# kjedrzejewski/video-cycle_gan-upscaling

Hardware: AMD Instinct MI355X
Metric: upscaled frames/s (train step, G+D fwd+bwd) at 256->512 (higher is better)
Workload: dtype f32; 1 GPU; C2: make_upscaler_orig((512,512,3),k=3,x2,res=9) + PatchGAN-70, batch 8/GPU, gan2 wiring, Wasserstein + pixel-MSE, faithful 3-call step incl. predict pass; global_batch=8, frame=256x256->512x512, parallelism=dp1, launch=hipGraph replay

## Files before the change

### video-cycle_gan-upscaling_amd/csrc/conv_wgrad.hip

```cpp
#include "vcg_common.hpp"

namespace {

struct WgradParams {
    const float* A;
    const float* B;
    float* part;
    float* dbpart;
    int n, mtot, ah, aw;
    int jctot, bh, bw;
    int pt, pl, flip;
    int jc;
    int m_blocks, j_blocks, slabs;
    int tiles_x, tiles_y, tiles_total, tiles_per_slab;
    int m_pad, j_pad;
};

template <int S, int NW, int NJ, int MW, int TH, int KH, int KW>
struct WgCfg {
    static constexpr int T = KH * KW;
    static constexpr int NT = 64 * NW;
    static constexpr int JTILES = (MW == 2 ? NW : NW / 2) * NJ;
    static constexpr int JCMAX = (JTILES * 32) / T;
    static constexpr int AST = TH * 32 + 1;
    static constexpr int BH = (TH - 1) * S + KH;
    static constexpr int BW = 31 * S + KW;
    static constexpr int round_to(int v, int r) { return v + ((r - v % 32) % 32 + 32) % 32; }
    static constexpr int BRS = round_to(BW, KW % 32);
    static constexpr int BPS = round_to(BH * BRS, T % 32);
    static constexpr int A_ELEMS = 64 * TH * 32;
    static constexpr int B_ELEMS = JCMAX * BH * BW;
    static constexpr int A_PT = (A_ELEMS + NT - 1) / NT;
    static constexpr int RG = NT / 32;
    static constexpr int ROWS = JCMAX * BH;
    static constexpr int QSEG = BW / 32, REM = BW % 32;
    static constexpr int RPT = (ROWS + RG - 1) / RG;
    static constexpr int HPT = (ROWS * REM + NT - 1) / NT;
    static constexpr int REMD = REM > 0 ? REM : 1;
    static constexpr int B_PT = RPT * QSEG + HPT;
    static constexpr size_t LDS_BYTES = ((size_t)64 * AST + (size_t)JCMAX * BPS + 64) * sizeof(float);
};

template <int S, int NW, int NJ, int MW, int TH, int KH, int KW>
__global__ __launch_bounds__(64 * NW, (MW * NJ * 16 > 100 ? 1 : 2)) void wgrad_kernel(const WgradParams p) {
    using C = WgCfg<S, NW, NJ, MW, TH, KH, KW>;
    extern __shared__ __attribute__((aligned(16))) float smem[];
    float* s_a = smem;
    float* s_b = smem + 64 * C::AST;

    const int tid = threadIdx.x, lane = tid & 63, wv = tid >> 6;
    const int half = lane >> 5, l31 = lane & 31;
    int b = blockIdx.x;
    const int jb = b % p.j_blocks; b /= p.j_blocks;
    const int mb = b % p.m_blocks; b /= p.m_blocks;
    const int slab = b;
    const int m0 = mb * 64, jc0 = jb * p.jc;
    const int jc_here = min(p.jc, p.jctot - jc0);
    const int jvalid = jc_here * C::T;

    int boff[NJ];
#pragma unroll
    for (int i = 0; i < NJ; ++i) {
        const int j = ((MW == 2 ? wv : (wv >> 1)) * NJ + i) * 32 + l31;
        int o = 0;
        if (j < jvalid) {
            const int jc = j / C::T, t = j % C::T;
            int ky = t / KW, kx = t % KW;
            if (p.flip) { ky = KH - 1 - ky; kx = KW - 1 - kx; }
            o = jc * C::BPS + ky * C::BRS + kx;
        }
        boff[i] = o + half * S;
    }
    const float* ap0 = s_a + ((MW == 2 ? 0 : (wv & 1)) * 32 + l31) * C::AST + half;

    f32x16 acc[MW][NJ];
#pragma unroll
    for (int m = 0; m < MW; ++m)
#pragma unroll
        for (int i = 0; i < NJ; ++i)
#pragma unroll
            for (int r = 0; r < 16; ++r) acc[m][i][r] = 0.f;
    float dbacc = 0.f;
    const bool do_db = p.dbpart != nullptr && jb == 0 && wv == 0;

    const int t_begin = slab * p.tiles_per_slab;
    const int t_end = min(t_begin + p.tiles_per_slab, p.tiles_total);

    float ra[C::A_PT], rb[C::B_PT];
    auto load_tile = [&](int tile) {
        int q = tile;
        const int tx = q % p.tiles_x; q /= p.tiles_x;
        const int ty = q % p.tiles_y; q /= p.tiles_y;
        const int n = q;
        const int ax0 = tx * 32, ay0 = ty * TH;
        const vcg_rsrc rA = make_rsrc(p.A + (size_t)n * p.mtot * p.ah * p.aw, (size_t)p.mtot * p.ah * p.aw * sizeof(float));
#pragma unroll
        for (int i = 0; i < C::A_PT; ++i) {
            const int e = tid + i * C::NT;
            const int c = e & 31, r = (e >> 5) % TH, m = e / (32 * TH);
            const int ay = ay0 + r, ax = ax0 + c;
            const bool ok = e < C::A_ELEMS && m0 + m < p.mtot && ay < p.ah && ax < p.aw;
            ra[i] = buf_load(rA, ok ? 4u * (unsigned)(((m0 + m) * p.ah + ay) * p.aw + ax) : VCG_OOB);
        }
        const vcg_rsrc rB = make_rsrc(p.B + ((size_t)n * p.jctot + jc0) * p.bh * p.bw, (size_t)(p.jctot - jc0) * p.bh * p.bw * sizeof(float));
        const int by0 = ay0 * S - p.pt, bx0 = ax0 * S - p.pl;
        const int c32 = tid & 31, rg = tid >> 5;
#pragma unroll
        for (int i = 0; i < C::RPT; ++i) {
            const int row = rg + i * C::RG;
            const int jc = row / C::BH, r = row % C::BH;
            const int by = by0 + r;
            const bool rok = row < C::ROWS && jc < jc_here && by >= 0 && by < p.bh;
            const int rbase = (jc * p.bh + by) * p.bw + bx0;
#pragma unroll
            for (int q = 0; q < C::QSEG; ++q) {
                const int bx = bx0 + q * 32 + c32;
                const bool ok = rok && bx >= 0 && bx < p.bw;
                rb[i * C::QSEG + q] = buf_load(rB, ok ? 4u * (unsigned)(rbase + q * 32 + c32) : VCG_OOB);
            }
        }
#pragma unroll
        for (int i = 0; i < C::HPT; ++i) {
            const int e = tid + i * C::NT;
            const int row = e / C::REMD, c = C::QSEG * 32 + e % C::REMD;
            const int jc = row / C::BH, r = row % C::BH;
            const int by = by0 + r, bx = bx0 + c;
            const bool ok = row < C::ROWS && jc < jc_here && by >= 0 && by < p.bh && bx >= 0 && bx < p.bw;
            rb[C::RPT * C::QSEG + i] = buf_load(rB, ok ? 4u * (unsigned)((jc * p.bh + by) * p.bw + bx) : VCG_OOB);
        }
    };
    auto store_tile = [&]() {
#pragma unroll
        for (int i = 0; i < C::A_PT; ++i) {
            const int e = tid + i * C::NT;
            if (e < C::A_ELEMS) {
                const int c = e & 31, r = (e >> 5) % TH, m = e / (32 * TH);
                s_a[m * C::AST + r * 32 + c] = ra[i];
            }
        }
        const int c32 = tid & 31, rg = tid >> 5;
#pragma unroll
        for (int i = 0; i < C::RPT; ++i) {
            const int row = rg + i * C::RG;
            if (row < C::ROWS) {
                const int jc = row / C::BH, r = row % C::BH;
#pragma unroll
                for (int q = 0; q < C::QSEG; ++q) s_b[jc * C::BPS + r * C::BRS + q * 32 + c32] = rb[i * C::QSEG + q];
            }
        }
#pragma unroll
        for (int i = 0; i < C::HPT; ++i) {
            const int e = tid + i * C::NT;
            const int row = e / C::REMD, c = C::QSEG * 32 + e % C::REMD;
            if (row < C::ROWS) {
                const int jc = row / C::BH, r = row % C::BH;
                s_b[jc * C::BPS + r * C::BRS + c] = rb[C::RPT * C::QSEG + i];
            }
        }
    };

    if (t_begin < t_end) load_tile(t_begin);
    for (int tile = t_begin; tile < t_end; ++tile) {
        __syncthreads();
        store_tile();
        __syncthreads();
        if (tile + 1 < t_end) load_tile(tile + 1);
        if (do_db) {
            const float* row = s_a + lane * C::AST;
#pragma unroll
            for (int i = 0; i < TH * 32; ++i) dbacc += row[i];
        }
#pragma unroll
        for (int r = 0; r < TH; ++r) {
#pragma unroll
            for (int st = 0; st < 16; ++st) {
                float av[MW];
#pragma unroll
                for (int m = 0; m < MW; ++m) av[m] = ap0[m * 32 * C::AST + r * 32 + 2 * st];
#pragma unroll
                for (int i = 0; i < NJ; ++i) {
                    const float bv = s_b[boff[i] + (r * S) * C::BRS + 2 * st * S];
#pragma unroll
                    for (int m = 0; m < MW; ++m) acc[m][i] = mfma32(av[m], bv, acc[m][i]);
                }
            }
        }
    }

    float* out = p.part + ((size_t)slab * p.m_pad + m0 + (MW == 2 ? 0 : (wv & 1)) * 32) * p.j_pad + (size_t)jb * (C::JTILES * 32);
#pragma unroll
    for (int m = 0; m < MW; ++m)
#pragma unroll
        for (int i = 0; i < NJ; ++i) {
            const int jcol = ((MW == 2 ? wv : (wv >> 1)) * NJ + i) * 32 + l31;
#pragma unroll
            for (int r = 0; r < 16; ++r) out[(size_t)(m * 32 + mfma_row(r, lane)) * p.j_pad + jcol] = acc[m][i][r];
        }
    if (do_db) p.dbpart[(size_t)slab * p.m_pad + m0 + lane] = dbacc;
}

struct ReduceParams {
    const float* part;
    const float* dbpart;
    float* dw;
    float* db;
    int slabs, m_pad, j_pad, mtot, jctot, jc, jbw, T;
    int ts, sm, sj;
};

__global__ __launch_bounds__(256) void wgrad_reduce_kernel(const ReduceParams p) {
    const size_t idx = (size_t)blockIdx.x * 256 + threadIdx.x;
    const size_t total = (size_t)p.m_pad * p.j_pad;
    if (idx >= total) return;
    const int m = (int)(idx / p.j_pad), jg = (int)(idx % p.j_pad);
    if (m >= p.mtot) return;
    const int jb = jg / p.jbw, jl = jg % p.jbw;
    if (jl >= p.jc * p.T) return;
    const int jc = jb * p.jc + jl / p.T, t = jl % p.T;
    if (jc >= p.jctot) return;
    float s8[8] = {0.f, 0.f, 0.f, 0.f, 0.f, 0.f, 0.f, 0.f};
    const float* src = p.part + idx;
    int k = 0;
    for (; k + 8 <= p.slabs; k += 8) {
#pragma unroll
        for (int u = 0; u < 8; ++u) s8[u] += src[(size_t)(k + u) * total];
    }
#pragma unroll
    for (int u = 0; u < 8; ++u)
        if (k + u < p.slabs) s8[u] += src[(size_t)(k + u) * total];
    const float s = ((s8[0] + s8[1]) + (s8[2] + s8[3])) + ((s8[4] + s8[5]) + (s8[6] + s8[7]));
    p.dw[(size_t)t * p.ts + (size_t)m * p.sm + (size_t)jc * p.sj] = s;
}

__global__ __launch_bounds__(256) void wgrad_db_reduce_kernel(const float* dbpart, float* db, int slabs, int m_pad, int mtot) {
    __shared__ float red[4][64];
    const int c = threadIdx.x & 63, g = threadIdx.x >> 6;
    const int m = blockIdx.x * 64 + c;
    float s4[4] = {0.f, 0.f, 0.f, 0.f};
    if (m < mtot) {
        int k = g;
        for (; k + 12 < slabs; k += 16) {
#pragma unroll
            for (int u = 0; u < 4; ++u) s4[u] += dbpart[(size_t)(k + 4 * u) * m_pad + m];
        }
        for (; k < slabs; k += 4) s4[0] += dbpart[(size_t)k * m_pad + m];
    }
    red[g][c] = (s4[0] + s4[1]) + (s4[2] + s4[3]);
    __syncthreads();
    if (g == 0 && m < mtot) db[m] = (red[0][c] + red[1][c]) + (red[2][c] + red[3][c]);
}

struct Plan {
    int S, NW, NJ, MW, TH, KH, KW, jc, m_blocks, j_blocks, slabs, tiles_x, tiles_y, tiles_total, tiles_per_slab;
    int m_pad, j_pad;
    size_t ws_part_bytes, ws_bytes;
    bool ok;
};

inline void pick_layout(int KH, int KW, int S, int jtot, int* nw, int* nj, int* mw) {
    *mw = 2;
    if (jtot <= 64) { *nw = 2; *nj = 1; return; }
    if (KH != KW) { *nw = 4; *nj = 2; return; }
    switch (KH) {
        case 1: *nw = 4; *nj = 2; return;
        case 3: if (jtot <= 256) { *nw = 4; *nj = 2; } else { *nw = 4; *nj = 9; *mw = 1; } return;
        case 4: if (S == 2) { *nw = 4; *nj = 2; } else { *nw = 4; *nj = 8; *mw = 1; } return;
        case 5: if (jtot <= 256 || S == 3) { *nw = 4; *nj = 2; } else { *nw = 4; *nj = 13; *mw = 1; } return;
        case 9: *nw = 4; *nj = 2; return;
        default: *nw = 0; *nj = 0; return;
    }
}

Plan make_plan(int n, int mtot, int ah, int aw, int jctot, int kh, int kw, int S) {
    Plan pl{};
    pl.ok = false;
    if (S < 1 || S > 3 || (S == 3 && (kh != 5 || kw != 5)) || (kh == 9 && S != 1)) return pl;
    if (kh != kw && (S != 1 || (kh != 1 && kw != 1))) return pl;
    if (kh == 1 && kw == 1 && S != 1) return pl;
    const int T = kh * kw;
    pl.S = S; pl.KH = kh; pl.KW = kw;
    pl.TH = (S == 1) ? 2 : 1;
    pick_layout(kh, kw, S, jctot * T, &pl.NW, &pl.NJ, &pl.MW);
    if (pl.NW == 0) return pl;
    const int cap = (pl.MW == 2 ? pl.NW : pl.NW / 2) * pl.NJ * 32;
    pl.jc = cap / T;
    if (pl.jc < 1) return pl;
    if (pl.jc > jctot) pl.jc = jctot;
    pl.m_blocks = ceil_div(mtot, 64);
    pl.j_blocks = ceil_div(jctot, pl.jc);
    pl.tiles_x = ceil_div(aw, 32);
    pl.tiles_y = ceil_div(ah, pl.TH);
    pl.tiles_total = pl.tiles_x * pl.tiles_y * n;
    int slabs = ceil_div(pl.MW == 1 ? 256 : 768, pl.m_blocks * pl.j_blocks);
    if (slabs > pl.tiles_total) slabs = pl.tiles_total;
    if (slabs < 1) slabs = 1;
    pl.tiles_per_slab = ceil_div(pl.tiles_total, slabs);
    pl.slabs = ceil_div(pl.tiles_total, pl.tiles_per_slab);
    pl.m_pad = pl.m_blocks * 64;
    pl.j_pad = pl.j_blocks * cap;
    pl.ws_part_bytes = align_up((size_t)pl.slabs * pl.m_pad * pl.j_pad * sizeof(float), 256);
    pl.ws_bytes = pl.ws_part_bytes + (size_t)pl.slabs * pl.m_pad * sizeof(float);
    pl.ok = true;
    return pl;
}

template <int S, int NW, int NJ, int MW, int TH, int KH, int KW>
int launch_wgrad(const WgradParams& p, int grid, hipStream_t st) {
    using C = WgCfg<S, NW, NJ, MW, TH, KH, KW>;
    static_assert(C::LDS_BYTES <= 160 * 1024, "wgrad tile does not fit the 160 KiB LDS");
    auto kern = wgrad_kernel<S, NW, NJ, MW, TH, KH, KW>;
    if (int e = vcg_allow_dyn_lds(reinterpret_cast<const void*>(kern), C::LDS_BYTES)) return e;
    hipLaunchKernelGGL(kern, dim3(grid), dim3(C::NT), C::LDS_BYTES, st, p);
    VCG_LAUNCH_CHECK();
    return VCG_OK;
}

}

size_t vcg_internal_wgrad_ws(int n, int mtot, int ah, int aw, int jctot, int kh, int kw, int S) {
    Plan pl = make_plan(n, mtot, ah, aw, jctot, kh, kw, S);
    return pl.ok ? pl.ws_bytes : 0;
}

int vcg_internal_wgrad(const float* A, const float* B, float* dw, float* db, int n, int mtot, int ah, int aw,
                       int jctot, int bh, int bw, int kh, int kw, int S, int pt, int pl_, int flip, int ts, int sm,
                       int sj, void* ws, size_t ws_bytes, hipStream_t st) {
    Plan pl = make_plan(n, mtot, ah, aw, jctot, kh, kw, S);
    if (!pl.ok) return VCG_E_UNSUPPORTED;
    if (ws == nullptr || ws_bytes < pl.ws_bytes) return VCG_E_WORKSPACE;
    WgradParams p{};
    p.A = A; p.B = B; p.part = (float*)ws;
    p.dbpart = db ? (float*)((char*)ws + pl.ws_part_bytes) : nullptr;
    p.n = n; p.mtot = mtot; p.ah = ah; p.aw = aw; p.jctot = jctot; p.bh = bh; p.bw = bw;
    p.pt = pt; p.pl = pl_; p.flip = flip; p.jc = pl.jc;
    p.m_blocks = pl.m_blocks; p.j_blocks = pl.j_blocks; p.slabs = pl.slabs;
    p.tiles_x = pl.tiles_x; p.tiles_y = pl.tiles_y; p.tiles_total = pl.tiles_total;
    p.tiles_per_slab = pl.tiles_per_slab;
    p.m_pad = pl.m_pad; p.j_pad = pl.j_pad;
    const int grid = pl.slabs * pl.m_blocks * pl.j_blocks;
    int rc = VCG_E_UNSUPPORTED;
#define VCG_WG2(S_, NW_, NJ_, MW_, TH_, KH_, KW_)                                                                        \
    if (S == S_ && pl.NW == NW_ && pl.NJ == NJ_ && pl.MW == MW_ && pl.KH == KH_ && pl.KW == KW_ && pl.TH == TH_) \
    rc = launch_wgrad<S_, NW_, NJ_, MW_, TH_, KH_, KW_>(p, grid, st)
#define VCG_WG(S_, NW_, NJ_, MW_, TH_, K_) VCG_WG2(S_, NW_, NJ_, MW_, TH_, K_, K_)
    VCG_WG(1, 2, 1, 2, 2, 3); VCG_WG(1, 4, 2, 2, 2, 3); VCG_WG(1, 4, 9, 1, 2, 3);
    VCG_WG(2, 2, 1, 2, 1, 3); VCG_WG(2, 4, 2, 2, 1, 3); VCG_WG(2, 4, 9, 1, 1, 3);
    VCG_WG(1, 2, 1, 2, 2, 4); VCG_WG(1, 4, 8, 1, 2, 4);
    VCG_WG(2, 2, 1, 2, 1, 4); VCG_WG(2, 4, 2, 2, 1, 4);
    VCG_WG(1, 4, 2, 2, 2, 5); VCG_WG(1, 4, 13, 1, 2, 5);
    VCG_WG(2, 4, 2, 2, 1, 5); VCG_WG(2, 4, 13, 1, 1, 5);
    VCG_WG(3, 4, 2, 2, 1, 5);
    VCG_WG(1, 4, 2, 2, 2, 9);
    VCG_WG(1, 2, 1, 2, 2, 1); VCG_WG(1, 4, 2, 2, 2, 1);
    VCG_WG2(1, 2, 1, 2, 2, 1, 3); VCG_WG2(1, 4, 2, 2, 2, 1, 3); VCG_WG2(1, 2, 1, 2, 2, 3, 1); VCG_WG2(1, 4, 2, 2, 2, 3, 1);
    VCG_WG2(1, 2, 1, 2, 2, 1, 5); VCG_WG2(1, 4, 2, 2, 2, 1, 5); VCG_WG2(1, 2, 1, 2, 2, 5, 1); VCG_WG2(1, 4, 2, 2, 2, 5, 1);
    VCG_WG2(1, 2, 1, 2, 2, 1, 7); VCG_WG2(1, 4, 2, 2, 2, 1, 7); VCG_WG2(1, 2, 1, 2, 2, 7, 1); VCG_WG2(1, 4, 2, 2, 2, 7, 1);
#undef VCG_WG2
#undef VCG_WG
    if (rc != VCG_OK) return rc;
    ReduceParams r{};
    r.part = (const float*)ws; r.dbpart = p.dbpart; r.dw = dw; r.db = db;
    r.slabs = pl.slabs; r.m_pad = pl.m_pad; r.j_pad = pl.j_pad;
    r.mtot = mtot; r.jctot = jctot; r.jc = pl.jc; r.jbw = (pl.MW == 2 ? pl.NW : pl.NW / 2) * pl.NJ * 32; r.T = kh * kw;
    r.ts = ts; r.sm = sm; r.sj = sj;
    const size_t total = (size_t)pl.m_pad * pl.j_pad;
    hipLaunchKernelGGL(wgrad_reduce_kernel, dim3((unsigned)((total + 255) / 256)), dim3(256), 0, st, r);
    VCG_LAUNCH_CHECK();
    if (db != nullptr) {
        hipLaunchKernelGGL(wgrad_db_reduce_kernel, dim3(ceil_div(mtot, 64)), dim3(256), 0, st, (const float*)p.dbpart, db,
                           pl.slabs, pl.m_pad, mtot);
        VCG_LAUNCH_CHECK();
    }
    return VCG_OK;
}
```

Measured before the change: 127.0 frames/s.

## Add warp-specialized wgrad kernel with dedicated loader waves and double-buffered LDS

For MW==1 configurations, the weight-gradient conv kernel becomes a warp-specialized one. Two loader waves stream A/B tiles from global memory into a double-buffered LDS stage, while four MFMA waves compute from the other stage with software-pipelined LDS reads. Bias-gradient accumulation moves into registers during loading, replacing the per-tile LDS row sum. The aim is to overlap global loads with the MFMA work and drop the serialized load/store/sync phases. The trade-offs are double the LDS footprint, which may limit occupancy, and extra compile-time stamp instrumentation that is off by default.

```diff
diff --git a/video-cycle_gan-upscaling_amd/csrc/conv_wgrad.hip b/video-cycle_gan-upscaling_amd/csrc/conv_wgrad.hip
--- a/video-cycle_gan-upscaling_amd/csrc/conv_wgrad.hip
+++ b/video-cycle_gan-upscaling_amd/csrc/conv_wgrad.hip
@@ -1,6 +1,37 @@
 #include "vcg_common.hpp"
 
 namespace {
+
+#ifdef VCG_WGRAD_STAMPS
+constexpr int WGF_SLOTS = 10;
+__device__ unsigned long long vcg_wgrad_stamp_sums[256 * 6 * WGF_SLOTS];
+#define WGF_STAMP(t)                                                                  \
+    do {                                                                              \
+        __builtin_amdgcn_sched_barrier(0);                                            \
+        asm volatile("s_memtime %0\n\ts_waitcnt lgkmcnt(0)" : "=s"(t)::"memory");     \
+        __builtin_amdgcn_sched_barrier(0);                                            \
+    } while (0)
+#define WGF_ADD(i, a, b) wgf_s[i] += (b) - (a)
+#define WGF_VMWAIT() __builtin_amdgcn_s_waitcnt(0x0F70)
+#define WGF_BEGIN()                                                                   \
+    unsigned long long wgf_s[WGF_SLOTS] = {0, 0, 0, 0, 0, 0, 0, 0, 0, 0}, wgf_a, wgf_b; \
+    const unsigned long long wgf_k0 = __builtin_amdgcn_s_memtime();                   \
+    __builtin_amdgcn_s_waitcnt(0xC07F)
+#define WGF_END(wave)                                                                 \
+    do {                                                                              \
+        if ((threadIdx.x & 63) == 0 && blockIdx.x < 256) {                            \
+            wgf_s[8] = __builtin_amdgcn_s_memtime() - wgf_k0;                         \
+            unsigned long long* o = vcg_wgrad_stamp_sums + (blockIdx.x * 6 + (wave)) * WGF_SLOTS; \
+            for (int i = 0; i < WGF_SLOTS; ++i) o[i] = wgf_s[i];                      \
+        }                                                                             \
+    } while (0)
+#else
+#define WGF_STAMP(t) do { } while (0)
+#define WGF_ADD(i, a, b) do { } while (0)
+#define WGF_VMWAIT() do { } while (0)
+#define WGF_BEGIN() do { } while (0)
+#define WGF_END(wave) do { } while (0)
+#endif
 
 struct WgradParams {
     const float* A;
@@ -81,7 +112,13 @@
 #pragma unroll
             for (int r = 0; r < 16; ++r) acc[m][i][r] = 0.f;
     float dbacc = 0.f;
-    const bool do_db = p.dbpart != nullptr && jb == 0 && wv == 0;
+    constexpr bool DB_REGS = MW == 1;
+    constexpr int DBSTEP = C::NT / (32 * TH);
+    static_assert(!DB_REGS || C::A_ELEMS % C::NT == 0, "wgrad: whole A passes");
+    const bool do_db = p.dbpart != nullptr && jb == 0 && (DB_REGS || wv == 0);
+    float dbl[DB_REGS ? C::A_PT : 1];
+#pragma unroll
+    for (int i = 0; i < (DB_REGS ? C::A_PT : 1); ++i) dbl[i] = 0.f;
 
     const int t_begin = slab * p.tiles_per_slab;
     const int t_end = min(t_begin + p.tiles_per_slab, p.tiles_total);
@@ -137,6 +174,7 @@
                 const int c = e & 31, r = (e >> 5) % TH, m = e / (32 * TH);
                 s_a[m * C::AST + r * 32 + c] = ra[i];
             }
+            if constexpr (DB_REGS) dbl[i] += ra[i];
         }
         const int c32 = tid & 31, rg = tid >> 5;
 #pragma unroll
@@ -159,17 +197,26 @@
         }
     };
 
+    WGF_BEGIN();
     if (t_begin < t_end) load_tile(t_begin);
     for (int tile = t_begin; tile < t_end; ++tile) {
+        WGF_STAMP(wgf_a);
         __syncthreads();
+        WGF_STAMP(wgf_b); WGF_ADD(0, wgf_a, wgf_b);
+        WGF_VMWAIT();
+        WGF_STAMP(wgf_a); WGF_ADD(1, wgf_b, wgf_a);
         store_tile();
+        WGF_STAMP(wgf_b); WGF_ADD(2, wgf_a, wgf_b);
         __syncthreads();
+        WGF_STAMP(wgf_a); WGF_ADD(3, wgf_b, wgf_a);
         if (tile + 1 < t_end) load_tile(tile + 1);
-        if (do_db) {
+        WGF_STAMP(wgf_b); WGF_ADD(4, wgf_a, wgf_b);
+        if (!DB_REGS && do_db) {
             const float* row = s_a + lane * C::AST;
 #pragma unroll
             for (int i = 0; i < TH * 32; ++i) dbacc += row[i];
         }
+        WGF_STAMP(wgf_a); WGF_ADD(5, wgf_b, wgf_a);
 #pragma unroll
         for (int r = 0; r < TH; ++r) {
 #pragma unroll
@@ -185,7 +232,9 @@
                 }
             }
         }
-    }
+        WGF_STAMP(wgf_b); WGF_ADD(6, wgf_a, wgf_b); WGF_ADD(7, 0, 1);
+    }
+    WGF_END(wv);
 
     float* out = p.part + ((size_t)slab * p.m_pad + m0 + (MW == 2 ? 0 : (wv & 1)) * 32) * p.j_pad + (size_t)jb * (C::JTILES * 32);
 #pragma unroll
@@ -196,7 +245,264 @@
 #pragma unroll
             for (int r = 0; r < 16; ++r) out[(size_t)(m * 32 + mfma_row(r, lane)) * p.j_pad + jcol] = acc[m][i][r];
         }
-    if (do_db) p.dbpart[(size_t)slab * p.m_pad + m0 + lane] = dbacc;
+    if constexpr (DB_REGS) {
+        if (do_db) {
+#pragma unroll
+            for (int i = 0; i < C::A_PT; ++i) {
+                float v = dbl[i];
+#pragma unroll
+                for (int o = 16; o > 0; o >>= 1) v += __shfl_xor(v, o, 64);
+                if (TH == 2) v += __shfl_xor(v, 32, 64);
+                if ((lane & 31) == 0 && (TH == 1 || lane == 0)) p.dbpart[(size_t)slab * p.m_pad + m0 + (tid >> 5) / TH + i * DBSTEP] = v;
+            }
+        }
+    } else {
+        if (do_db) p.dbpart[(size_t)slab * p.m_pad + m0 + lane] = dbacc;
+    }
+}
+
+template <int S, int NJ, int TH, int KH, int KW>
+struct WgLdrCfg {
+    using C = WgCfg<S, 4, NJ, 1, TH, KH, KW>;
+    static constexpr int NMUL = 4, NLDR = 2;
+    static constexpr int NT = 64 * (NMUL + NLDR);
+    static constexpr int NTL = 64 * NLDR;
+    static constexpr int STAGE = (64 * C::AST + C::JCMAX * C::BPS + 3) / 4 * 4;
+    static constexpr size_t LDS_BYTES = 2 * (size_t)STAGE * sizeof(float);
+    static constexpr int A_PT = C::A_ELEMS / NTL;
+    static constexpr int MSTEP = NTL / (32 * TH);
+    static constexpr int BW0 = C::BW < 64 ? C::BW : 64;
+    static constexpr int REM = C::BW - BW0, REMD = REM > 0 ? REM : 1;
+    static constexpr int RPW = (C::ROWS + NLDR - 1) / NLDR;
+    static constexpr int CH = 32;
+    static constexpr int HPT = (C::ROWS * REM + NTL - 1) / NTL;
+    static constexpr bool PIPE = 16 * NJ + 3 * NJ + 2 <= 224;
+    static_assert(TH == 1 || TH == 2, "wgrad loaders: A rows of 32 or 64 floats");
+    static_assert(C::A_ELEMS % NTL == 0 && C::BW <= 128, "wgrad loaders: piece shapes");
+};
+
+template <int S, int NJ, int TH, int KH, int KW, int LW>
+__device__ __forceinline__ void wgrad_loader_wave(const WgradParams& p, float* smem, int lane, int m0, int jc0, int jc_here,
+                                                  float* dbout, int t_begin, int t_end) {
+    using C = WgCfg<S, 4, NJ, 1, TH, KH, KW>;
+    using L = WgLdrCfg<S, NJ, TH, KH, KW>;
+    __builtin_amdgcn_s_setprio(3);
+    const int ltid = LW * 64 + lane;
+    const int ac = ltid & 31, ar = (ltid >> 5) % TH, am = (ltid >> 5) / TH;
+    const int a_lane = (am * p.ah + ar) * p.aw + ac;
+    const int a_step = L::MSTEP * p.ah * p.aw;
+    const int a_lds = am * C::AST + ar * 32 + ac;
+    const int a_rows = (p.mtot - m0 - am + L::MSTEP - 1) / L::MSTEP;
+    const size_t a_img = (size_t)p.mtot * p.ah * p.aw, b_img = (size_t)p.jctot * p.bh * p.bw;
+    const int b_plane = p.bh * p.bw;
+    float dbl[L::A_PT];
+#pragma unroll
+    for (int i = 0; i < L::A_PT; ++i) dbl[i] = 0.f;
+
+    int tx = t_begin % p.tiles_x, ty = (t_begin / p.tiles_x) % p.tiles_y, n = t_begin / p.tiles_x / p.tiles_y;
+    WGF_BEGIN();
+
+    auto stage = [&](float* st) {
+        const int ax0 = tx * 32, ay0 = ty * TH;
+        const vcg_rsrc rA = make_rsrc(p.A + (size_t)n * a_img, a_img * sizeof(float));
+        const vcg_rsrc rB = make_rsrc(p.B + (size_t)n * b_img + (size_t)jc0 * b_plane, (size_t)jc_here * b_plane * sizeof(float));
+        {
+            const unsigned a_off = 4u * (unsigned)((m0 * p.ah + ay0) * p.aw + ax0 + a_lane);
+            const unsigned a_ok = (ay0 + ar < p.ah && ax0 + ac < p.aw) ? ~0u : 0u;
+            float ra[L::A_PT];
+            WGF_STAMP(wgf_a);
+#pragma unroll
+            for (int i = 0; i < L::A_PT; ++i) {
+                const unsigned mk = a_ok & (unsigned)((i - a_rows) >> 31);
+                ra[i] = buf_load(rA, ((a_off + 4u * (unsigned)(i * a_step)) & mk) | (VCG_OOB & ~mk));
+            }
+            WGF_STAMP(wgf_b); WGF_ADD(4, wgf_a, wgf_b);
+            WGF_VMWAIT();
+            WGF_STAMP(wgf_a); WGF_ADD(1, wgf_b, wgf_a);
+#pragma unroll
+            for (int i = 0; i < L::A_PT; ++i) {
+                st[a_lds + i * L::MSTEP * C::AST] = ra[i];
+                dbl[i] += ra[i];
+            }
+            WGF_STAMP(wgf_b); WGF_ADD(2, wgf_a, wgf_b);
+        }
+        const int by0 = ay0 * S - p.pt, bx0 = ax0 * S - p.pl;
+        const int b_tile = by0 * p.bw + bx0;
+        const bool colok = lane < L::BW0 && (unsigned)(bx0 + lane) < (unsigned)p.bw;
+        unsigned b_off[C::BH], b_ok[C::BH], b_bad[C::BH];
+#pragma unroll
+        for (int r = 0; r < C::BH; ++r) {
+            b_off[r] = 4u * (unsigned)(b_tile + r * p.bw + lane);
+            b_ok[r] = (colok && (unsigned)(by0 + r) < (unsigned)p.bh) ? ~0u : 0u;
+            b_bad[r] = VCG_OOB & ~b_ok[r];
+        }
+        float* sb = st + 64 * C::AST;
+#pragma unroll
+        for (int c0 = 0; c0 < L::RPW; c0 += L::CH) {
+            float rb[L::CH];
+            WGF_STAMP(wgf_a);
+#pragma unroll
+            for (int k = 0; k < L::CH; ++k) {
+                const int row = (c0 + k) * L::NLDR + LW, jc = row / C::BH, r = row % C::BH;
+                if (c0 + k < L::RPW && row < C::ROWS)
+                    rb[k] = buf_load(rB, ((b_off[r] + 4u * (unsigned)(jc * b_plane)) & b_ok[r]) | b_bad[r]);
+            }
+            WGF_STAMP(wgf_b); WGF_ADD(4, wgf_a, wgf_b);
+            WGF_VMWAIT();
+            WGF_STAMP(wgf_a); WGF_ADD(1, wgf_b, wgf_a);
+            if (lane < L::BW0) {
+#pragma unroll
+                for (int k = 0; k < L::CH; ++k) {
+                    const int row = (c0 + k) * L::NLDR + LW, jc = row / C::BH, r = row % C::BH;
+                    if (c0 + k < L::RPW && row < C::ROWS) sb[jc * C::BPS + r * C::BRS + lane] = rb[k];
+                }
+            }
+            WGF_STAMP(wgf_b); WGF_ADD(2, wgf_a, wgf_b);
+        }
+        if constexpr (L::REM > 0) {
+            float rr[L::HPT];
+#pragma unroll
+            for (int i = 0; i < L::HPT; ++i) {
+                const int e = ltid + i * L::NTL;
+                const int row = e / L::REMD, c = 64 + e % L::REMD;
+                const int jc = row / C::BH, r = row % C::BH;
+                const bool ok = row < C::ROWS && jc < jc_here && (unsigned)(by0 + r) < (unsigned)p.bh && (unsigned)(bx0 + c) < (unsigned)p.bw;
+                rr[i] = buf_load(rB, ok ? 4u * (unsigned)(b_tile + jc * b_plane + r * p.bw + c) : VCG_OOB);
+            }
+#pragma unroll
+            for (int i = 0; i < L::HPT; ++i) {
+                const int e = ltid + i * L::NTL;
+                const int row = e / L::REMD, c = 64 + e % L::REMD;
+                if (row < C::ROWS) sb[(row / C::BH) * C::BPS + (row % C::BH) * C::BRS + c] = rr[i];
+            }
+        }
+        if (++tx == p.tiles_x) {
+            tx = 0;
+            if (++ty == p.tiles_y) { ty = 0; ++n; }
+        }
+    };
+
+    stage(smem);
+    int buf = 0;
+    for (int tile = t_begin; tile < t_end; ++tile, buf ^= 1) {
+        WGF_STAMP(wgf_a);
+        lds_barrier();
+        WGF_STAMP(wgf_b); WGF_ADD(0, wgf_a, wgf_b); WGF_ADD(7, 0, 1);
+        if (tile + 1 < t_end) stage(smem + (buf ^ 1) * L::STAGE);
+    }
+    WGF_END(4 + LW);
+
+    if (dbout != nullptr) {
+#pragma unroll
+        for (int i = 0; i < L::A_PT; ++i) {
+            float v = dbl[i];
+#pragma unroll
+            for (int o = 16; o > 0; o >>= 1) v += __shfl_xor(v, o, 64);
+            if (TH == 2) v += __shfl_xor(v, 32, 64);
+            if ((lane & 31) == 0 && (TH == 1 || lane == 0)) dbout[am + i * L::MSTEP] = v;
+        }
+    }
+}
+
+template <int S, int NJ, int TH, int KH, int KW>
+__global__ __launch_bounds__(384, 1) void wgrad_ldr_kernel(const WgradParams p) {
+    using C = WgCfg<S, 4, NJ, 1, TH, KH, KW>;
+    using L = WgLdrCfg<S, NJ, TH, KH, KW>;
+    extern __shared__ __attribute__((aligned(16))) float smem[];
+
+    const int tid = threadIdx.x, lane = tid & 63;
+    const int wv = __builtin_amdgcn_readfirstlane(tid >> 6);
+    const int half = lane >> 5, l31 = lane & 31;
+    int b = blockIdx.x;
+    const int jb = b % p.j_blocks; b /= p.j_blocks;
+    const int mb = b % p.m_blocks; b /= p.m_blocks;
+    const int slab = b;
+    const int m0 = mb * 64, jc0 = jb * p.jc;
+    const int jc_here = min(p.jc, p.jctot - jc0);
+    const int jvalid = jc_here * C::T;
+    const int t_begin = slab * p.tiles_per_slab;
+    const int t_end = min(t_begin + p.tiles_per_slab, p.tiles_total);
+
+    if (wv >= L::NMUL) {
+        float* dbout = (p.dbpart != nullptr && jb == 0) ? p.dbpart + (size_t)slab * p.m_pad + m0 : nullptr;
+        if (wv == L::NMUL)
+            wgrad_loader_wave<S, NJ, TH, KH, KW, 0>(p, smem, lane, m0, jc0, jc_here, dbout, t_begin, t_end);
+        else
+            wgrad_loader_wave<S, NJ, TH, KH, KW, 1>(p, smem, lane, m0, jc0, jc_here, dbout, t_begin, t_end);
+        return;
+    }
+
+    int boff[NJ];
+#pragma unroll
+    for (int i = 0; i < NJ; ++i) {
+        const int j = ((wv >> 1) * NJ + i) * 32 + l31;
+        int o = 0;
+        if (j < jvalid) {
+            const int jc = j / C::T, t = j % C::T;
+            int ky = t / KW, kx = t % KW;
+            if (p.flip) { ky = KH - 1 - ky; kx = KW - 1 - kx; }
+            o = jc * C::BPS + ky * C::BRS + kx;
+        }
+        boff[i] = 64 * C::AST + o + half * S;
+    }
+    int aoff = ((wv & 1) * 32 + l31) * C::AST + half;
+    int flip_stage = L::STAGE;
+
+    f32x16 acc[NJ];
+#pragma unroll
+    for (int i = 0; i < NJ; ++i)
+#pragma unroll
+        for (int r = 0; r < 16; ++r) acc[i][r] = 0.f;
+
+    WGF_BEGIN();
+    for (int tile = t_begin; tile < t_end; ++tile) {
+        WGF_STAMP(wgf_a);
+        lds_barrier();
+        WGF_STAMP(wgf_b); WGF_ADD(0, wgf_a, wgf_b);
+        if constexpr (L::PIPE) {
+            float av[2], bv[2][NJ];
+            av[0] = smem[aoff];
+#pragma unroll
+            for (int i = 0; i < NJ; ++i) bv[0][i] = smem[boff[i]];
+#pragma unroll
+            for (int k = 0; k < TH * 16; ++k) {
+                if (k + 1 < TH * 16) {
+                    const int r = (k + 1) / 16, s = (k + 1) % 16;
+                    av[(k + 1) & 1] = smem[aoff + r * 32 + 2 * s];
+#pragma unroll
+                    for (int i = 0; i < NJ; ++i) bv[(k + 1) & 1][i] = smem[boff[i] + (r * S) * C::BRS + 2 * s * S];
+                }
+                __builtin_amdgcn_sched_barrier(0);
+#pragma unroll
+                for (int i = 0; i < NJ; ++i) acc[i] = mfma32(av[k & 1], bv[k & 1][i], acc[i]);
+                __builtin_amdgcn_sched_barrier(0);
+            }
+        } else {
+#pragma unroll
+            for (int r = 0; r < TH; ++r) {
+#pragma unroll
+                for (int s = 0; s < 16; ++s) {
+                    const float av = smem[aoff + r * 32 + 2 * s];
+#pragma unroll
+                    for (int i = 0; i < NJ; ++i) acc[i] = mfma32(av, smem[boff[i] + (r * S) * C::BRS + 2 * s * S], acc[i]);
+                }
+            }
+        }
+        WGF_STAMP(wgf_a); WGF_ADD(6, wgf_b, wgf_a); WGF_ADD(7, 0, 1);
+        aoff += flip_stage;
+#pragma unroll
+        for (int i = 0; i < NJ; ++i) boff[i] += flip_stage;
+        flip_stage = -flip_stage;
+    }
+    WGF_END(wv);
+
+    float* out = p.part + ((size_t)slab * p.m_pad + m0 + (wv & 1) * 32) * p.j_pad + (size_t)jb * (C::JTILES * 32);
+#pragma unroll
+    for (int i = 0; i < NJ; ++i) {
+        const int jcol = ((wv >> 1) * NJ + i) * 32 + l31;
+#pragma unroll
+        for (int r = 0; r < 16; ++r) out[(size_t)mfma_row(r, lane) * p.j_pad + jcol] = acc[i][r];
+    }
 }
 
 struct ReduceParams {
@@ -306,13 +612,27 @@
 
 template <int S, int NW, int NJ, int MW, int TH, int KH, int KW>
 int launch_wgrad(const WgradParams& p, int grid, hipStream_t st) {
-    using C = WgCfg<S, NW, NJ, MW, TH, KH, KW>;
-    static_assert(C::LDS_BYTES <= 160 * 1024, "wgrad tile does not fit the 160 KiB LDS");
-    auto kern = wgrad_kernel<S, NW, NJ, MW, TH, KH, KW>;
-    if (int e = vcg_allow_dyn_lds(reinterpret_cast<const void*>(kern), C::LDS_BYTES)) return e;
-    hipLaunchKernelGGL(kern, dim3(grid), dim3(C::NT), C::LDS_BYTES, st, p);
-    VCG_LAUNCH_CHECK();
-    return VCG_OK;
+#if !defined(VCG_WGRAD_STAMPS_SINGLE) && !defined(VCG_EXP_SINGLE)
+    if constexpr (MW == 1) {
+        static_assert(NW == 4, "wgrad loaders: four multiplying waves");
+        using L = WgLdrCfg<S, NJ, TH, KH, KW>;
+        static_assert(L::LDS_BYTES <= 160 * 1024, "two wgrad stages do not fit the 160 KiB LDS");
+        auto kern = wgrad_ldr_kernel<S, NJ, TH, KH, KW>;
+        if (int e = vcg_allow_dyn_lds(reinterpret_cast<const void*>(kern), L::LDS_BYTES)) return e;
+        hipLaunchKernelGGL(kern, dim3(grid), dim3(L::NT), L::LDS_BYTES, st, p);
+        VCG_LAUNCH_CHECK();
+        return VCG_OK;
+    } else
+#endif
+    {
+        using C = WgCfg<S, NW, NJ, MW, TH, KH, KW>;
+        static_assert(C::LDS_BYTES <= 160 * 1024, "wgrad tile does not fit the 160 KiB LDS");
+        auto kern = wgrad_kernel<S, NW, NJ, MW, TH, KH, KW>;
+        if (int e = vcg_allow_dyn_lds(reinterpret_cast<const void*>(kern), C::LDS_BYTES)) return e;
+        hipLaunchKernelGGL(kern, dim3(grid), dim3(C::NT), C::LDS_BYTES, st, p);
+        VCG_LAUNCH_CHECK();
+        return VCG_OK;
+    }
 }
 
 }
@@ -373,3 +693,10 @@
     }
     return VCG_OK;
 }
+
+#ifdef VCG_WGRAD_STAMPS
+extern "C" int vcg_debug_wgrad_stamps(unsigned long long* host_out) {
+    if (hipDeviceSynchronize() != hipSuccess) return -1;
+    return (int)hipMemcpyFromSymbol(host_out, HIP_SYMBOL(vcg_wgrad_stamp_sums), sizeof(unsigned long long) * 256 * 6 * WGF_SLOTS);
+}
+#endif
```

Result: no change. 126.4 frames/s (-0.4%).
